# xinyiW915/ReLaX-VQA

Measured on AMD Instinct MI355X. Metric: clips/sec (32 sampled frames, 1080p) feature extraction, higher is better.
Workload: dtype f32 (fp32-grade split-operand arithmetic, fp32 accumulate: the whole ViT (GEMMs and attention), ResNet-50's stem, layer3 / layer4, and in layer1 / layer2 the 3x3 convolutions, every conv3 (back to back with its 3x3), the downsample convolutions and layer2's conv1 on fp32 operands as 2 fp16 planes x

## Files before the change

### relax-vqa_amd/csrc/gemm_h2.hip

```cpp
#include "relax_internal.h"
#include "host_logic.h"
#include "h2.h"
#include "gelu.h"

#ifndef H3_EP_FETCH_AHEAD
#define H3_EP_FETCH_AHEAD 0
#endif
#ifndef H2_STAMP
#define H2_STAMP(i_)
#define H2_STAMPS_BEFORE_LAUNCH(h_, p_, units_)
#define H2_STAMPS_AFTER_LAUNCH(h_, p_, units_, s_)
#endif
#ifndef H3_ABL_NO_A
#define H3_ABL_NO_A(taps_, perimg_, p_) false
#define H3_ABL_NO_OUT_H2(taps_, p_) false
#endif
#ifndef H3_KSTEP
#define H3_KSTEP(k_) (k_)
#endif

namespace relax {

typedef float h2k_f32x4 __attribute__((ext_vector_type(4)));
typedef float f32x4 __attribute__((ext_vector_type(4)));
// ... 168 lines not shown
    {
        const int per_group = p.group_m * p.tiles_n;
        const int g = tile / per_group;
        const int first = g * p.group_m;
        const int gsz = p.tiles_m - first < p.group_m ? p.tiles_m - first : p.group_m;
        const int w = tile - g * per_group;
        tm = first + w % gsz;
        tn = w / gsz;
    }
    const int m0 = tm * BM;
    const int n0 = tn * BN;
    H2_STAMP(0);

    const int64_t row_bytes = (int64_t)p.K * 4;
    __amdgpu_buffer_rsrc_t rsrc_a, rsrc_w;
    {
        const int64_t left = (int64_t)(p.M - m0) * row_bytes;
        rsrc_a = __builtin_amdgcn_make_buffer_rsrc(const_cast<char*>(p.a + (int64_t)m0 * row_bytes), 0,
                                                   (int)(left < kH2MaxRecords ? left : kH2MaxRecords), 0x00020000);
        rsrc_w = __builtin_amdgcn_make_buffer_rsrc(const_cast<char*>(p.w + (int64_t)n0 * row_bytes), 0, (int)(BN * row_bytes), 0x00020000);
    }
    unsigned voff_a, voff_w;
    {
        const int r = 32 * wave + (lane >> 1);
        voff_a = m0 + r < p.M ? (unsigned)(r * (int)row_bytes + (lane & 1) * 16) : kH2OutOfRange;
        voff_w = (unsigned)(r * (int)row_bytes + (lane & 1) * 16);
    }
    int d_kt = kt_begin;
#define H2_ISSUE_PIECE(st_, j_)                                                                                         \
    {                                                                                                                   \
        const int soff_ = d_kt * kH2ChunkBytes + ((j_) >> 1) * 32;                                                      \
        const int dst_ = (st_) * STAGE + ((j_) >> 1) * (STAGE / 2) + ((j_) & 1) * (BM * 32) + wave * 1024;               \
        if (((j_) & 1) == 0) { H2_DMA(rsrc_a, dst_, voff_a, soff_); }                                                    \
        else { H2_DMA(rsrc_w, dst_, voff_w, soff_); }                                                                    \
    }
#define H2_ISSUE(st_)                                                                                                   \
    {                                                                                                                   \
        _Pragma("unroll") for (int j = 0; j < PPW; ++j) H2_ISSUE_PIECE(st_, j);                                         \
        ++d_kt;                                                                                                         \
    }

    floatx4 acc[8][4];
#pragma unroll
    for (int i = 0; i < 8; ++i)
#pragma unroll
        for (int j = 0; j < 4; ++j)
#pragma unroll
            for (int r = 0; r < 4; ++r) acc[i][j][r] = 0.f;

    const int r16 = lane & 15, g16 = lane >> 4;
    const int a_hl = (g16 >> 1) * (STAGE / 2) + (wm * 128 + r16) * 32 + ((g16 & 1) << 4);
    const int b_hh = (BM + wn * 64 + r16) * 32 + ((g16 & 1) << 4);
    h2k_f16x8 xb[2][4][2], ya[2];
#define H2_READ_XB(set_, sp_)                                                                                           \
    _Pragma("unroll") for (int y = 0; y < 4; ++y) {                                                                     \
        xb[set_][y][0] = *reinterpret_cast<const h2k_f16x8*>((sp_) + b_hh + y * 16 * 32);                               \
        xb[set_][y][1] = *reinterpret_cast<const h2k_f16x8*>((sp_) + b_hh + y * 16 * 32 + STAGE / 2);                   \
    }
#define H2_READ_A(buf_, e_, sp_)                                                                                        \
    {                                                                                                                   \
        ya[buf_] = *reinterpret_cast<const h2k_f16x8*>((sp_) + a_hl + (e_) * 16 * 32);                                  \
        __builtin_amdgcn_sched_barrier(0);                        \
    }
#define H2_MFMAS(set_, buf_, e_)                                                                                        \
    {                                                                                                                   \
        _Pragma("unroll") for (int y = 0; y < 4; ++y)                                                                   \
            acc[e_][y] = __builtin_amdgcn_mfma_f32_16x16x32_f16(ya[buf_], xb[set_][y][1], acc[e_][y], 0, 0, 0);         \
        _Pragma("unroll") for (int y = 0; y < 4; ++y)                                                                   \
            acc[e_][y] = __builtin_amdgcn_mfma_f32_16x16x32_f16(ya[buf_], xb[set_][y][0], acc[e_][y], 0, 0, 0);         \
        __builtin_amdgcn_sched_barrier(0);        \
    }
#define H2_REGION(xs_, st_, has_next_, has_d_)                                                                          \
    {                                                                                                                   \
        const char* sn_ = smem + (((st_) + 1) % NSTG) * STAGE;                                                          \
        if (has_next_) {                                                                                                \
            if (has_d_) asm volatile("s_waitcnt vmcnt(%0) lgkmcnt(0)" ::"n"((NSTG - 2) * PPW) : "memory");              \
            else asm volatile("s_waitcnt vmcnt(0) lgkmcnt(0)" ::: "memory");                                            \
            __builtin_amdgcn_s_barrier();                                                                               \
            H2_READ_XB((xs_) ^ 1, sn_);                                                                                 \
            H2_READ_A(0, 0, sn_);                                                                                       \
        }                                                                                                               \
        H2_MFMAS(xs_, 1, 7);                                                                                            \
        if (has_next_) {                                                                                                \
            _Pragma("unroll") for (int e = 0; e < 7; ++e) {                                                             \
                H2_READ_A((e + 1) & 1, e + 1, sn_);                                                                     \
                if ((has_d_) && e < PPW) H2_ISSUE_PIECE(st_, e);                                                        \
                H2_MFMAS((xs_) ^ 1, e & 1, e);                                                                          \
            }                                                                                                           \
            if (has_d_) ++d_kt;                                                                                         \
        }                                                                                                               \
    }

    const int nk = kt_end - kt_begin;
    {
        const int pre = nk < NSTG ? nk : NSTG;
        for (int i = 0; i < pre; ++i) H2_ISSUE(i);
        if (pre >= 4) asm volatile("s_waitcnt vmcnt(%0)" ::"n"(3 * PPW) : "memory");
        else if (pre == 3) asm volatile("s_waitcnt vmcnt(%0)" ::"n"(2 * PPW) : "memory");
        else if (pre == 2) asm volatile("s_waitcnt vmcnt(%0)" ::"n"(PPW) : "memory");
        else asm volatile("s_waitcnt vmcnt(0)" ::: "memory");
    }
    __builtin_amdgcn_s_barrier();
    H2_READ_XB(0, smem);
    H2_READ_A(0, 0, smem);
    H2_STAMP(1);
#pragma unroll
    for (int e = 0; e < 7; ++e) {
        H2_READ_A((e + 1) & 1, e + 1, smem);
        H2_MFMAS(0, e & 1, e);
    }
    {
        constexpr int PERIOD = (NSTG % 2 == 0) ? NSTG : 2 * NSTG;
        int k = 0;
        for (; k + PERIOD + NSTG <= nk; k += PERIOD) {
#pragma unroll
            for (int i = 0; i < PERIOD; ++i) H2_REGION(i & 1, i % NSTG, true, true);
        }
        for (; k < nk; k += PERIOD) {
#pragma unroll
            for (int i = 0; i < PERIOD; ++i)
                if (k + i < nk) H2_REGION(i & 1, i % NSTG, k + i + 1 < nk, k + i + NSTG < nk);
        }
    }
#undef H2_REGION
#undef H2_MFMAS
#undef H2_READ_A
#undef H2_READ_XB
#undef H2_ISSUE
#undef H2_ISSUE_PIECE
    H2_STAMP(2);
    __syncthreads();

    float* stg = reinterpret_cast<float*>(smem);
    constexpr int LDC = BN + 4;
    constexpr int EP_ROWS = 64;
    constexpr int C8 = BN / 8;
    constexpr int NT = 512;
    static_assert(EP_ROWS * LDC * 4 <= NSTG * STAGE, "epilogue pass must fit the staging LDS");
    constexpr int EP_STEP = NT / C8;
    constexpr int EP_ITERS = EP_ROWS / EP_STEP;
    const bool planes = p.out_h2 != nullptr;
    const int lcA = planes ? (tid % C8) * 8 : (tid % C8) * 4;
    const int lcB = planes ? lcA + 4 : lcA + BN / 2;
    const int lr0 = tid / C8;
    const f32x4 zero4 = {0.f, 0.f, 0.f, 0.f};
    f32x4 bias_a = zero4, bias_b = zero4, cs_a = zero4, cs_b = zero4;
    if (slice < 0) {
        cs_a = *reinterpret_cast<const f32x4*>(p.colscale + n0 + lcA);
        cs_b = *reinterpret_cast<const f32x4*>(p.colscale + n0 + lcB);
        if (p.bias) {
            bias_a = *reinterpret_cast<const f32x4*>(p.bias + n0 + lcA);
            bias_b = *reinterpret_cast<const f32x4*>(p.bias + n0 + lcB);
        }
    }
    const bool interior = m0 + BM <= p.M;
#pragma unroll
    for (int pass = 0; pass < BM / EP_ROWS; ++pass) {
        if (pass > 0) __syncthreads();
        f32x4 ra[EP_ITERS], rb[EP_ITERS];
        float rs[EP_ITERS];
#pragma unroll
        for (int it = 0; it < EP_ITERS; ++it) {
            const int m = m0 + pass * EP_ROWS + it * EP_STEP + lr0;
            ra[it] = zero4;
            rb[it] = zero4;
            rs[it] = 1.f;
            if (slice < 0 && (interior || m < p.M)) {
                if (p.residual) {
                    const float* r = p.residual + (int64_t)m * p.N + n0;
                    ra[it] = *reinterpret_cast<const f32x4*>(r + lcA);
                    rb[it] = *reinterpret_cast<const f32x4*>(r + lcB);
                }
                if (p.rowscale) rs[it] = p.rowscale[m];
            }
        }
#pragma unroll
        for (int x = 0; x < 8; ++x) {
            const int rb0 = wm * 128 + x * 16;
            if (rb0 / EP_ROWS == pass) {
#pragma unroll
                for (int y = 0; y < 4; ++y)
#pragma unroll
                    for (int r = 0; r < 4; ++r) stg[(rb0 % EP_ROWS + 4 * g16 + r) * LDC + wn * 64 + y * 16 + r16] = acc[x][y][r];
            }
        }
        __syncthreads();
#pragma unroll
        for (int it = 0; it < EP_ITERS; ++it) {
            const int lr = it * EP_STEP + lr0;
            const int trow = pass * EP_ROWS + lr;
            const int m = m0 + trow;
            if (!interior && m >= p.M) continue;
            f32x4 va = *reinterpret_cast<const f32x4*>(stg + lr * LDC + lcA);
            f32x4 vb = *reinterpret_cast<const f32x4*>(stg + lr * LDC + lcB);
            if (slice >= 0) {
                float* o = p.partial + ((int64_t)split_tile * p.nsplit + slice) * (BM * BN) + (int64_t)trow * BN;
                *reinterpret_cast<f32x4*>(o + lcA) = va;
                *reinterpret_cast<f32x4*>(o + lcB) = vb;
                continue;
            }
            va = va * (cs_a * rs[it]) + bias_a;
            vb = vb * (cs_b * rs[it]) + bias_b;
            if (p.residual) {
                va += ra[it];
                vb += rb[it];
            }
            if (p.act == 1) {
                va = (f32x4){fmaxf(va.x, 0.f), fmaxf(va.y, 0.f), fmaxf(va.z, 0.f), fmaxf(va.w, 0.f)};
                vb = (f32x4){fmaxf(vb.x, 0.f), fmaxf(vb.y, 0.f), fmaxf(vb.z, 0.f), fmaxf(vb.w, 0.f)};
            } else if (p.act == 2) {
                va = gelu_erf4(va);
                vb = gelu_erf4(vb);
            }
            const int64_t o = (int64_t)m * p.N + n0;
            if (p.out) {
                *reinterpret_cast<f32x4*>(p.out + o + lcA) = va;
                *reinterpret_cast<f32x4*>(p.out + o + lcB) = vb;
            }
            if (p.out_h2) store_h2_x8(p.out_h2 + (int64_t)m * ((int64_t)p.N * 4), n0 + lcA, va, vb, p.out_scale);
        }
    }
    H2_STAMP(3);
#endif
}

constexpr int H3_OPSTAGE = H2_BM * 128;
static_assert(H2_BM == H2_BN, "gemm_h3: the operand rings share their stage size");
#ifndef H3_PLAIN_STAGES
#define H3_PLAIN_STAGES 3, 2, 0
#endif
#ifndef H3_CONV1_STAGES
#define H3_CONV1_STAGES 2, 2, 0
#endif
#ifndef H3_TAPS_STAGES
#define H3_TAPS_STAGES 2, 2, 0
#endif
struct H3Rings { int a, b, order; };
constexpr H3Rings h3_rings(bool taps, bool perimg) { return taps ? H3Rings{H3_TAPS_STAGES} : perimg ? H3Rings{H3_CONV1_STAGES} : H3Rings{H3_PLAIN_STAGES}; }
constexpr size_t h3_lds_bytes(bool taps, bool perimg) { return (size_t)(h3_rings(taps, perimg).a + h3_rings(taps, perimg).b) * H3_OPSTAGE; }
#ifndef H2_STAMP_LATCH
#define H2_STAMP_LATCH(v_)
#define H2_STAMP_PUT(i_, v_)
#endif

__device__ inline float dpp_row_max(float v) {
#define H3_DPP_MAX(CTRL_) v = fmaxf(v, __builtin_bit_cast(float, __builtin_amdgcn_update_dpp(0, __builtin_bit_cast(int, v), CTRL_, 0xf, 0xf, true)))
    H3_DPP_MAX(0xB1);
    H3_DPP_MAX(0x4E);
    H3_DPP_MAX(0x141);
    H3_DPP_MAX(0x140);
#undef H3_DPP_MAX
    return v;
}

#if __HIP_DEVICE_COMPILE__
template <bool FOUR, bool TAPS, bool PERIMG, int ASTG, int BSTG, int ORDER>
__device__ __forceinline__ void gemm_h3_body(const H2Params& p) {
    constexpr int BM = H2_BM, BN = H2_BN, OPSTG = H3_OPSTAGE, IMG = OPSTG / 2, B0 = ASTG * OPSTG;
    constexpr int LA = ASTG - 2, LB = BSTG - 2;
    static_assert(LA >= 0 && LB >= 0 && LA + LB <= 1 && (ORDER == 0 || ORDER == 1), "gemm_h3: 2 + 2, 3 + 2 or 2 + 3 stages");
    constexpr int WAITN = ORDER == 0 ? 4 : 2;
    extern __shared__ __attribute__((aligned(16))) char smem[];
    const int tid = threadIdx.x;
    const int lane = tid & 63;
    const int wave = __builtin_amdgcn_readfirstlane(tid >> 6);
    const int wm = wave >> 2, wn = wave & 3;

    int tile, kt_begin, kt_end, slice = -1, split_tile = 0;
    {
        const int nk_all = p.K >> 5;
        const int b = blockIdx.x;
        if (b < p.full_tiles) {
            tile = xcd_remap_h2(b, p.full_tiles);
            kt_begin = 0;
            kt_end = nk_all;
        } else {
            const int u = b - p.full_tiles;
            split_tile = u / p.nsplit;
            slice = u - split_tile * p.nsplit;
            tile = p.full_tiles + split_tile;
            kt_begin = (int)((int64_t)nk_all * slice / p.nsplit);
            kt_end = (int)((int64_t)nk_all * (slice + 1) / p.nsplit);
        }
    }
    int tm, tn;
    {
        const int per_group = p.group_m * p.tiles_n;
        const int g = tile / per_group;
        const int first = g * p.group_m;
        const int gsz = p.tiles_m - first < p.group_m ? p.tiles_m - first : p.group_m;
        const int w = tile - g * per_group;
        tm = first + w % gsz;
        tn = w / gsz;
    }
    const int m0 = tm * BM;
    const int n0 = tn * BN;
#ifdef H3_STAGGER
    if (PERIMG && !TAPS && blockIdx.x < 256 && (blockIdx.x & 3)) {
        const unsigned long long t0 = __builtin_amdgcn_s_memtime(), wait = (unsigned long long)(blockIdx.x & 3) * (H3_STAGGER);
        while (__builtin_amdgcn_s_memtime() - t0 < wait) __builtin_amdgcn_s_sleep(32);
    }
#endif
    H2_STAMP(0);

    const int64_t row_bytes = (int64_t)p.K * 4;
    const int64_t arow_bytes = p.pixels ? (int64_t)p.Cin * 4 : row_bytes;
    const int img0 = p.pixels ? m0 / (p.Ho * p.Wo) : 0;
    __amdgpu_buffer_rsrc_t rsrc_a, rsrc_w;
    {
        const int64_t base = p.pixels ? (int64_t)img0 * p.H * p.W * arow_bytes : (int64_t)m0 * arow_bytes;
        const int64_t total = p.pixels ? (int64_t)(p.M / (p.Ho * p.Wo)) * p.H * p.W * arow_bytes : (int64_t)p.M * arow_bytes;
        const int64_t left = total - base;
        rsrc_a = __builtin_amdgcn_make_buffer_rsrc(const_cast<char*>(p.a + base), 0, (int)(left < kH2MaxRecords ? left : kH2MaxRecords), 0x00020000);
        rsrc_w = __builtin_amdgcn_make_buffer_rsrc(const_cast<char*>(p.w + (int64_t)n0 * row_bytes), 0, (int)(BN * row_bytes), 0x00020000);
    }
    unsigned voff[4];
    [[maybe_unused]] unsigned a_taps[2] = {0u, 0u};
    const int ntaps = TAPS ? p.K / p.Cin : 1;
#pragma unroll
    for (int q = 0; q < 4; ++q) {
        const int trow = (wave + 8 * q) * 16 + (lane >> 2);
        const int unit = (lane & 3) ^ ((4 - ((trow >> 2) & 3)) & 3);
        const int off = (unit >> 1) * kH2ChunkBytes + (unit & 1) * 16;
        if (q >= 2) {
            voff[q] = (unsigned)((trow - BM) * (int)row_bytes + off);
        } else if (m0 + trow >= p.M || H3_ABL_NO_A(TAPS, PERIMG, p)) {
            voff[q] = kH2OutOfRange;
        } else if (p.pixels) {
            const int m = m0 + trow;
            const int img = m / (p.Ho * p.Wo);
            const int rem = m - img * (p.Ho * p.Wo);
            const int oy = rem / p.Wo;
            const int ox = rem - oy * p.Wo;
            const int iy = oy * p.stride - p.pad, ix = ox * p.stride - p.pad;
            if (TAPS) {
                for (int t = 0, dy = 0, dx = 0; t < ntaps; ++t) {
                    if ((unsigned)(iy + dy) < (unsigned)p.H && (unsigned)(ix + dx) < (unsigned)p.W) a_taps[q] |= 1u << t;
                    if (++dx == p.KW) { dx = 0; ++dy; }
                }
            }
            voff[q] = (unsigned)((((img - img0) * p.H + iy) * p.W + ix) * (int)arow_bytes + off);
        } else {
            voff[q] = (unsigned)(trow * (int)arow_bytes + off);
        }
    }
    int dA_kt = kt_begin;
    [[maybe_unused]] int dA_cc = 0, dA_tap = 0, dA_dy = 0, dA_dx = 0;
    [[maybe_unused]] const int cin_chunks = p.Cin >> 4;
    if (TAPS) {
        dA_cc = kt_begin / ntaps;
        dA_tap = kt_begin - dA_cc * ntaps;
        dA_dy = dA_tap / p.KW;
        dA_dx = dA_tap - dA_dy * p.KW;
    }
    [[maybe_unused]] int dW_kt_own = dA_kt, dW_cc_own = dA_cc, dW_tap_own = dA_tap;
    int &dW_kt = LA + LB > 0 ? dW_kt_own : dA_kt, &dW_cc = LA + LB > 0 ? dW_cc_own : dA_cc, &dW_tap = LA + LB > 0 ? dW_tap_own : dA_tap;
#define H3_ISSUE_A(st_, i_)                                                                                             \
    {                                                                                                                   \
        const int dst_ = (st_) * OPSTG + ((i_) >> 1) * IMG + (wave + 8 * ((i_) & 1)) * 1024;                             \
        if (TAPS) {                                                                                                     \
            const bool ok_ = (a_taps[(i_) & 1] >> dA_tap) & 1u;                                                         \
            const int tapoff_ = (dA_dy * p.W + dA_dx) * (int)arow_bytes + dA_cc * (2 * kH2ChunkBytes) + ((i_) >> 1) * 32; \
            H2_DMA(rsrc_a, dst_, ok_ ? voff[(i_) & 1] + (unsigned)tapoff_ : kH2OutOfRange, 0);                          \
        } else {                                                                                                        \
            H2_DMA(rsrc_a, dst_, voff[(i_) & 1], H3_KSTEP(dA_kt) * (2 * kH2ChunkBytes) + ((i_) >> 1) * 32);             \
        }                                                                                                               \
    }
#define H3_ISSUE_W(st_, i_)                                                                                             \
    {                                                                                                                   \
        const int dst_ = B0 + (st_) * OPSTG + ((i_) >> 1) * IMG + (wave + 8 * ((i_) & 1)) * 1024;                        \
        const int wk_ = TAPS ? (dW_tap * cin_chunks + 2 * dW_cc) * kH2ChunkBytes : H3_KSTEP(dW_kt) * (2 * kH2ChunkBytes); \
        H2_DMA(rsrc_w, dst_, voff[2 + ((i_) & 1)], wk_ + ((i_) >> 1) * 32);                                              \
    }
#define H3_ADVANCE_A()                                                                                                  \
    {                                                                                                                   \
        ++dA_kt;                                                                                                        \
        if (TAPS) {                                                                                                     \
            ++dA_tap;                                                                                                   \
            ++dA_dx;                                                                                                    \
            const bool wx_ = dA_dx == p.KW;                                                                             \
            dA_dx = wx_ ? 0 : dA_dx;                                                                                    \
            dA_dy += wx_ ? 1 : 0;                                                                                       \
            const bool wt_ = dA_tap == ntaps;                                                                           \
            dA_tap = wt_ ? 0 : dA_tap;                                                                                  \
            dA_dy = wt_ ? 0 : dA_dy;                                                                                    \
            dA_cc += wt_ ? 1 : 0;                                                                                       \
        }                                                                                                               \
    }
#define H3_ADVANCE_W()                                                                                                  \
    if (LA + LB > 0) {                                                                                                  \
        ++dW_kt;                                                                                                        \
        if (TAPS) {                                                                                                     \
            ++dW_tap;                                                                                                   \
            const bool wt_ = dW_tap == ntaps;                                                                           \
            dW_tap = wt_ ? 0 : dW_tap;                                                                                  \
            dW_cc += wt_ ? 1 : 0;                                                                                       \
        }                                                                                                               \
    }
#define H3_ISSUE_SLOT(sa_, sb_, s_, has_a_, has_b_)                                                                     \
    {                                                                                                                   \
        const bool grouped_ = LA + LB > 0 && ORDER == 0;                                                                \
        const bool second_ = grouped_ ? (s_) >= 4 : ((s_) & 3) >= 2;                \
        const bool is_a_ = LA + LB == 0 ? !second_ : second_ == (LA == 1);      \
        const int i_ = grouped_ ? (s_) & 3 : ((s_) >> 2) * 2 + ((s_) & 1);                                              \
        if (is_a_) {                                                                                                    \
            if (has_a_) H3_ISSUE_A(sa_, i_);                                                                            \
        } else {                                                                                                        \
            if (has_b_) H3_ISSUE_W(sb_, i_);                                                                            \
        }                                                                                                               \
    }
#define H3_ISSUE_STEP_A(step_)                                                                                          \
    {                                                                                                                   \
        _Pragma("unroll") for (int i = 0; i < 4; ++i) H3_ISSUE_A((step_) % ASTG, i);                                    \
        H3_ADVANCE_A();                                                                                                 \
    }
#define H3_ISSUE_STEP_W(step_)                                                                                          \
    {                                                                                                                   \
        _Pragma("unroll") for (int i = 0; i < 4; ++i) H3_ISSUE_W((step_) % BSTG, i);                                    \
        H3_ADVANCE_W();                                                                                                 \
    }

    floatx4 acc[8][4];
#pragma unroll
    for (int i = 0; i < 8; ++i)
#pragma unroll
        for (int j = 0; j < 4; ++j)
#pragma unroll
            for (int r = 0; r < 4; ++r) acc[i][j][r] = 0.f;

    const int r16 = lane & 15, g16 = lane >> 4;
    const int f16 = (4 - ((r16 >> 2) & 3)) & 3;
    const int a_h = (wm * 128 + r16) * 64 + ((g16 ^ f16) << 4);
    const int b_h = (wn * 64 + r16) * 64 + ((g16 ^ f16) << 4);
    h2k_f16x8 xb[2][4][2], ya[2][2];
#define H3_READ_XB(set_, sp_)                                                                                           \
    _Pragma("unroll") for (int y = 0; y < 4; ++y) {                                                                     \
        xb[set_][y][0] = *reinterpret_cast<const h2k_f16x8*>((sp_) + b_h + y * 16 * 64);                                \
        xb[set_][y][1] = *reinterpret_cast<const h2k_f16x8*>((sp_) + b_h + y * 16 * 64 + IMG);                          \
    }
#define H3_READ_A(buf_, e_, sp_)                                                                                        \
    {                                                                                                                   \
        ya[buf_][0] = *reinterpret_cast<const h2k_f16x8*>((sp_) + a_h + (e_) * 16 * 64);                                \
        ya[buf_][1] = *reinterpret_cast<const h2k_f16x8*>((sp_) + a_h + (e_) * 16 * 64 + IMG);                          \
        __builtin_amdgcn_sched_barrier(0);                      \
    }
#define H3_MFMAS(set_, buf_, e_)                                                                                        \
    {                                                                                                                   \
        if (FOUR) {                                                                                                     \
            _Pragma("unroll") for (int y = 0; y < 4; ++y)                                                               \
                acc[e_][y] = __builtin_amdgcn_mfma_f32_16x16x32_f16(ya[buf_][1], xb[set_][y][1], acc[e_][y], 0, 0, 0);  \
        }                                                                                                               \
        _Pragma("unroll") for (int y = 0; y < 4; ++y)                                                                   \
            acc[e_][y] = __builtin_amdgcn_mfma_f32_16x16x32_f16(ya[buf_][1], xb[set_][y][0], acc[e_][y], 0, 0, 0);      \
        _Pragma("unroll") for (int y = 0; y < 4; ++y)                                                                   \
            acc[e_][y] = __builtin_amdgcn_mfma_f32_16x16x32_f16(ya[buf_][0], xb[set_][y][1], acc[e_][y], 0, 0, 0);      \
        _Pragma("unroll") for (int y = 0; y < 4; ++y)                                                                   \
            acc[e_][y] = __builtin_amdgcn_mfma_f32_16x16x32_f16(ya[buf_][0], xb[set_][y][0], acc[e_][y], 0, 0, 0);      \
        __builtin_amdgcn_sched_barrier(0);        \
    }
#define H3_REGION(k6_, has_next_, has_e_, has_l_)                                                                       \
    {                                                                                                                   \
        const char* sa_ = smem + (((k6_) + 1) % ASTG) * OPSTG;                                                          \
        const char* sb_ = smem + B0 + (((k6_) + 1) % BSTG) * OPSTG;                                                     \
        const bool has_a_ = LA ? (has_l_) : (has_e_), has_b_ = LB ? (has_l_) : (has_e_);                                \
        if (has_next_) {                                                                                                \
            if (LA + LB > 0 && (has_e_)) asm volatile("s_waitcnt vmcnt(%0) lgkmcnt(0)" ::"n"(WAITN) : "memory");        \
            else asm volatile("s_waitcnt vmcnt(0) lgkmcnt(0)" ::: "memory");                                            \
            __builtin_amdgcn_s_barrier();                                                                               \
            H3_READ_XB(((k6_) + 1) & 1, sb_);                                                                           \
            H3_READ_A(0, 0, sa_);                                                                                       \
            H3_ISSUE_SLOT(((k6_) + 2 + LA) % ASTG, ((k6_) + 2 + LB) % BSTG, 0, has_a_, has_b_);                         \
        }                                                                                                               \
        H3_MFMAS((k6_) & 1, 1, 7);                                                                                      \
        if (has_next_) {                                                                                                \
            _Pragma("unroll") for (int e = 0; e < 7; ++e) {                                                             \
                H3_READ_A((e + 1) & 1, e + 1, sa_);                                                                     \
                H3_ISSUE_SLOT(((k6_) + 2 + LA) % ASTG, ((k6_) + 2 + LB) % BSTG, e + 1, has_a_, has_b_);                 \
                H3_MFMAS(((k6_) + 1) & 1, e & 1, e);                                                                    \
            }                                                                                                           \
            if (has_a_) H3_ADVANCE_A();                                                                                 \
            if (has_b_) H3_ADVANCE_W();                                                                                 \
        }                                                                                                               \
    }

    const int nk = kt_end - kt_begin;
    if (LA + LB == 0) {
#pragma unroll
        for (int j = 0; j < 8; ++j) H3_ISSUE_SLOT(0, 0, j, true, true);
        H3_ADVANCE_A();
        H3_ADVANCE_W();
        if (nk > 1) {
#pragma unroll
            for (int j = 0; j < 8; ++j) H3_ISSUE_SLOT(1, 1, j, true, true);
            H3_ADVANCE_A();
            H3_ADVANCE_W();
            asm volatile("s_waitcnt vmcnt(8)" ::: "memory");
        } else {
            asm volatile("s_waitcnt vmcnt(0)" ::: "memory");
        }
    } else {
        if (LA) {
            H3_ISSUE_STEP_W(0);
            H3_ISSUE_STEP_A(0);
        } else {
            H3_ISSUE_STEP_A(0);
            H3_ISSUE_STEP_W(0);
        }
        if (nk > 1) {
            if (LA) {
                H3_ISSUE_STEP_W(1);
                H3_ISSUE_STEP_A(1);
            } else {
                H3_ISSUE_STEP_A(1);
                H3_ISSUE_STEP_W(1);
            }
        }
        if (nk > 2) {
            if (LA) H3_ISSUE_STEP_A(2) else H3_ISSUE_STEP_W(2)
            asm volatile("s_waitcnt vmcnt(12)" ::: "memory");
        } else if (nk > 1) {
            asm volatile("s_waitcnt vmcnt(8)" ::: "memory");
        } else {
            asm volatile("s_waitcnt vmcnt(0)" ::: "memory");
        }
    }
    __builtin_amdgcn_s_barrier();
    H3_READ_XB(0, smem + B0);
    H3_READ_A(0, 0, smem);
    H2_STAMP_LATCH(stamp1);
#pragma unroll
    for (int e = 0; e < 7; ++e) {
        H3_READ_A((e + 1) & 1, e + 1, smem);
        H3_MFMAS(0, e & 1, e);
    }
    {
        constexpr int PERIOD = LA + LB > 0 ? 6 : 2;
        int k = 0;
        for (; k + PERIOD + 1 + LA + LB < nk; k += PERIOD) {
#pragma unroll
            for (int i = 0; i < PERIOD; ++i) H3_REGION(i, true, true, true);
        }
        for (; k < nk; k += PERIOD) {
#pragma unroll
            for (int i = 0; i < PERIOD; ++i)
                if (k + i < nk) H3_REGION(i, k + i + 1 < nk, k + i + 2 < nk, k + i + 3 < nk);
        }
    }
#undef H3_REGION
#undef H3_ISSUE_STEP_W
#undef H3_ISSUE_STEP_A
#undef H3_ISSUE_SLOT
#undef H3_ADVANCE_W
#undef H3_ADVANCE_A
#undef H3_ISSUE_W
#undef H3_ISSUE_A
#undef H3_MFMAS
#undef H3_READ_A
#undef H3_READ_XB
    H2_STAMP_PUT(1, stamp1);
    H2_STAMP(2);
    __syncthreads();
    H2_STAMP(7);

    float* stg = reinterpret_cast<float*>(smem);
    constexpr int LDC = BN + 4;
    constexpr int EP_ROWS = 64;
    constexpr int C8 = BN / 8;
    constexpr int NT = 512;
    static_assert(EP_ROWS * LDC * 4 <= 96 * 1024 && 96 * 1024 + 64 <= (ASTG + BSTG) * OPSTG, "epilogue pass must fit the staging LDS");
    constexpr int EP_STEP = NT / C8;
    constexpr int EP_ITERS = EP_ROWS / EP_STEP;
    const bool planes = p.out_h2 != nullptr || (PERIMG && p.residual_h2 != nullptr);
    const int lcA = planes ? (tid % C8) * 8 : (tid % C8) * 4;
    const int lcB = planes ? lcA + 4 : lcA + BN / 2;
    const int lr0 = tid / C8;
    const f32x4 zero4 = {0.f, 0.f, 0.f, 0.f};
    const f32x4 cs_a = *reinterpret_cast<const f32x4*>(p.colscale + n0 + lcA);
    const f32x4 cs_b = *reinterpret_cast<const f32x4*>(p.colscale + n0 + lcB);
    const __amdgpu_buffer_rsrc_t rs_bias = __builtin_amdgcn_make_buffer_rsrc(const_cast<float*>(p.bias), 0, p.bias ? p.N * 4 : 0, 0x00020000);
    const f32x4 bias_a = __builtin_bit_cast(f32x4, __builtin_amdgcn_raw_buffer_load_b128(rs_bias, (n0 + lcA) * 4, 0, 0));
    const f32x4 bias_b = __builtin_bit_cast(f32x4, __builtin_amdgcn_raw_buffer_load_b128(rs_bias, (n0 + lcB) * 4, 0, 0));
    const bool interior = m0 + BM <= p.M;
    unsigned* simg = reinterpret_cast<unsigned*>(smem + 96 * 1024);
    const int rpi = p.rows_per_img;
    const int img_first = rpi > 0 ? m0 / rpi : 0;
    const int row_first = m0 - img_first * rpi;
    const float rpi_inv = rpi > 0 ? 1.f / (float)rpi : 0.f;
    auto img_of_row = [&](int trow) -> int {
        const int x = row_first + trow;
        int q = (int)((float)x * rpi_inv);
        q -= (q * rpi > x) ? 1 : 0;
        q += ((q + 1) * rpi <= x) ? 1 : 0;
        return img_first + q;
    };
    const bool lds_amax = PERIMG && p.amax_out && slice < 0 && p.rows_per_img >= 18;
    if (lds_amax && tid < 16) simg[tid] = 0u;
    const int64_t tile_ofs = ((int64_t)m0 * p.N + n0) * 4;
    const unsigned row_pitch = (unsigned)p.N * 4u;
    const unsigned ofs_f = (unsigned)lr0 * row_pitch + (unsigned)lcA * 4u;
    const unsigned ofs_p = (unsigned)lr0 * row_pitch + (unsigned)h2_offset(lcA);
    const unsigned ofs_fb = (unsigned)(lcB - lcA) * 4u;
    const bool res_planes = PERIMG && p.residual_h2 != nullptr;
    const char* res_ptr = res_planes ? p.residual_h2 : reinterpret_cast<const char*>(p.residual);
    const int64_t res_left = (int64_t)p.M * p.N * 4 - tile_ofs;
    const __amdgpu_buffer_rsrc_t rs_res = __builtin_amdgcn_make_buffer_rsrc(
        const_cast<char*>(res_ptr) + (res_ptr ? tile_ofs : 0), 0, (res_ptr && slice < 0) ? (int)(res_left < kH2MaxRecords ? res_left : kH2MaxRecords) : 0, 0x00020000);
    const unsigned ofs_r = res_planes ? ofs_p : ofs_f, ofs_rb = res_planes ? 32u : ofs_fb;
    char* tile_out = reinterpret_cast<char*>(p.out) + tile_ofs;
    char* tile_out_h2 = p.out_h2 + tile_ofs;
    f32x4 ra[EP_ITERS], rb[EP_ITERS];
    float rs[EP_ITERS], os[EP_ITERS], rri[EP_ITERS];
    int im[EP_ITERS];
#define H3_EP_FETCH(P_, IT_)                                                                                                     \
    {                                                                                                                            \
        const int trow_ = (P_) * EP_ROWS + (IT_) * EP_STEP + lr0;                                                                \
        const int m_ = m0 + trow_;                                                                                               \
        const unsigned row_ofs_ = (unsigned)(((P_) * EP_ROWS + (IT_) * EP_STEP) * row_pitch);                                    \
        ra[IT_] = __builtin_bit_cast(f32x4, __builtin_amdgcn_raw_buffer_load_b128(rs_res, row_ofs_ + ofs_r, 0, 0));              \
        rb[IT_] = __builtin_bit_cast(f32x4, __builtin_amdgcn_raw_buffer_load_b128(rs_res, row_ofs_ + ofs_r + ofs_rb, 0, 0));     \
        rs[IT_] = 1.f;                                                                                                           \
        os[IT_] = p.out_scale;                                                                                                   \
        rri[IT_] = 1.f;                                                                                                          \
        im[IT_] = 0;                                                                                                             \
        if (slice < 0 && (interior || m_ < p.M)) {                                                                               \
            if (p.rowscale) rs[IT_] = p.rowscale[m_];                                                                            \
            if (PERIMG && rpi > 0) {                                                      \
                im[IT_] = img_of_row(trow_);                                                                                     \
                if (p.img_in_inv) rs[IT_] = p.img_in_inv[im[IT_]];                                                               \
                if (p.img_out_scale) os[IT_] = p.img_out_scale[im[IT_]];                                                         \
            }                                                                                                                    \
            if (res_planes) rri[IT_] = p.img_res_inv[im[IT_]];  \
        }                                                                                                                        \
    }
    constexpr bool EP_AHEAD = PERIMG && H3_EP_FETCH_AHEAD;
    if constexpr (EP_AHEAD) {
#pragma unroll
        for (int it = 0; it < EP_ITERS; ++it) H3_EP_FETCH(0, it);
    }
#pragma unroll
    for (int pass = 0; pass < BM / EP_ROWS; ++pass) {
        if (pass > 0) __syncthreads();
        if constexpr (!EP_AHEAD) {
#pragma unroll
            for (int it = 0; it < EP_ITERS; ++it) H3_EP_FETCH(pass, it);
        }
        if (pass == 0) H2_STAMP(4);
#pragma unroll
        for (int x = 0; x < 8; ++x) {
            const int rb0 = wm * 128 + x * 16;
            if (rb0 / EP_ROWS == pass) {
#pragma unroll
                for (int y = 0; y < 4; ++y)
#pragma unroll
                    for (int r = 0; r < 4; ++r) stg[(rb0 % EP_ROWS + 4 * g16 + r) * LDC + wn * 64 + y * 16 + r16] = acc[x][y][r];
            }
        }
        __syncthreads();
        if (pass == 0) H2_STAMP(5);
        if constexpr (!EP_AHEAD) {
#pragma unroll
            for (int it = 0; it < EP_ITERS; ++it) {
                asm volatile("" : "+v"(ra[it]), "+v"(rb[it]), "+v"(rs[it]));
                if constexpr (PERIMG) asm volatile("" : "+v"(os[it]), "+v"(rri[it]));
            }
        }
#pragma unroll
        for (int it = 0; it < EP_ITERS; ++it) {
            const int lr = it * EP_STEP + lr0;
            const int trow = pass * EP_ROWS + lr;
            const int m = m0 + trow;
            f32x4 xa = ra[it], xb = rb[it];
            const float rs_it = rs[it], os_it = os[it];
            const int im_it = im[it];
            if (res_planes) {
                const h2_u32x4 hi = __builtin_bit_cast(h2_u32x4, xa), lo = __builtin_bit_cast(h2_u32x4, xb);
                const float ri = rri[it];
#define H2_LO16(u_) ((float)__builtin_bit_cast(_Float16, (unsigned short)((u_) & 0xffffu)))
#define H2_HI16(u_) ((float)__builtin_bit_cast(_Float16, (unsigned short)((u_) >> 16)))
                xa = (f32x4){H2_LO16(hi.x) + H2_LO16(lo.x), H2_HI16(hi.x) + H2_HI16(lo.x), H2_LO16(hi.y) + H2_LO16(lo.y),
                             H2_HI16(hi.y) + H2_HI16(lo.y)} * ri;
                xb = (f32x4){H2_LO16(hi.z) + H2_LO16(lo.z), H2_HI16(hi.z) + H2_HI16(lo.z), H2_LO16(hi.w) + H2_LO16(lo.w),
                             H2_HI16(hi.w) + H2_HI16(lo.w)} * ri;
#undef H2_LO16
#undef H2_HI16
            }
            if constexpr (EP_AHEAD) {
                if (pass + 1 < BM / EP_ROWS) H3_EP_FETCH(pass + 1, it);
            }
            if (!interior && m >= p.M) continue;
            f32x4 va = *reinterpret_cast<const f32x4*>(stg + lr * LDC + lcA);
            f32x4 vb = *reinterpret_cast<const f32x4*>(stg + lr * LDC + lcB);
            if (slice >= 0) {
                float* o = p.partial + ((int64_t)split_tile * p.nsplit + slice) * (BM * BN) + (int64_t)trow * BN;
                *reinterpret_cast<f32x4*>(o + lcA) = va;
                *reinterpret_cast<f32x4*>(o + lcB) = vb;
                continue;
            }
            va = va * (cs_a * rs_it) + bias_a;
            vb = vb * (cs_b * rs_it) + bias_b;
            if (res_ptr) {
                va += xa;
                vb += xb;
            }
            if (p.act == 1) {
                va = (f32x4){fmaxf(va.x, 0.f), fmaxf(va.y, 0.f), fmaxf(va.z, 0.f), fmaxf(va.w, 0.f)};
                vb = (f32x4){fmaxf(vb.x, 0.f), fmaxf(vb.y, 0.f), fmaxf(vb.z, 0.f), fmaxf(vb.w, 0.f)};
            } else if (p.act == 2) {
                va = gelu_erf4(va);
                vb = gelu_erf4(vb);
            }
            const unsigned row_ofs = (unsigned)((pass * EP_ROWS + it * EP_STEP) * row_pitch);
            if (p.out && (!PERIMG || m < p.out_rows)) {
                char* o = tile_out + (size_t)(unsigned)(row_ofs + ofs_f);
                *reinterpret_cast<f32x4*>(o) = va;
                *reinterpret_cast<f32x4*>(o + ofs_fb) = vb;
            }
            if (PERIMG && p.gap) {
                *reinterpret_cast<f32x4*>(stg + lr * LDC + lcA) = va;
                *reinterpret_cast<f32x4*>(stg + lr * LDC + lcB) = vb;
            }
            if (p.out_h2 && !H3_ABL_NO_OUT_H2(TAPS, p)) {
                h2_u32x4 hi, lo;
                split2_x8(va * os_it, vb * os_it, hi, lo);
                char* o = tile_out_h2 + (size_t)(unsigned)(row_ofs + ofs_p);
                *reinterpret_cast<h2_u32x4*>(o) = hi;
                *reinterpret_cast<h2_u32x4*>(o + 32) = lo;
            }
            if (PERIMG && p.amax_out) {
                float mx = fmaxf(fmaxf(fmaxf(va.x, va.y), fmaxf(va.z, va.w)), fmaxf(fmaxf(vb.x, vb.y), fmaxf(vb.z, vb.w)));
                mx = dpp_row_max(mx);
                if ((tid & 15) == 0) {
                    if (lds_amax) atomicMax(simg + (im_it - img_first), __float_as_uint(mx));
                    else atomicMax(p.amax_out + im_it, __float_as_uint(mx));
                }
            }
        }
        if (pass == 0) H2_STAMP(6);
        if (PERIMG && p.gap && slice < 0) {
            __syncthreads();
            for (int e = tid; e < (EP_ROWS / 4) * BN; e += NT) {
                const int g = e / BN, col = e - g * BN;
                const int mg = m0 + pass * EP_ROWS + g * 4;
                if (mg < p.gap_rows) {
                    float t = 0.f;
#pragma unroll
                    for (int r = 0; r < 4; ++r) t += stg[(g * 4 + r) * LDC + col];
                    p.gap[(int64_t)(mg >> 2) * p.N + n0 + col] = t;
                }
            }
        }
    }
#undef H3_EP_FETCH
    if (lds_amax) {
        __syncthreads();
        if (tid < 16 && simg[tid] != 0u) atomicMax(p.amax_out + img_first + tid, simg[tid]);
    }
    H2_STAMP(3);
}
#endif

template <bool FOUR, bool TAPS = false, bool PERIMG = false>
__global__ __launch_bounds__(512, 2) void gemm_h3(const H2Params p) {
#if __HIP_DEVICE_COMPILE__
    constexpr H3Rings R = h3_rings(TAPS, PERIMG);
    gemm_h3_body<FOUR, TAPS, PERIMG, R.a, R.b, R.order>(p);
#endif
}

__global__ __launch_bounds__(256) void splitk_finish_h2(const H2Params p) {
    constexpr int BM = H2_BM, BN = H2_BN;
    const int split_tile = blockIdx.y;
    const int tile = p.full_tiles + split_tile;
    int tm, tn;
    {
        const int per_group = p.group_m * p.tiles_n;
        const int g = tile / per_group;
        const int first = g * p.group_m;
        const int gsz = p.tiles_m - first < p.group_m ? p.tiles_m - first : p.group_m;
        const int w = tile - g * per_group;
        tm = first + w % gsz;
        tn = w / gsz;
    }
    const int m0 = tm * BM;
    const int n0 = tn * BN;
    const int e8 = blockIdx.x * 256 + threadIdx.x;
    const int lr = e8 / (BN / 8), lc = (e8 % (BN / 8)) * 8;
    const int m = m0 + lr;
    __shared__ unsigned s_mx[8];
    const int img_b0 = p.rows_per_img > 0 ? (m0 + blockIdx.x * 8) / p.rows_per_img : 0;
    if (threadIdx.x < 8) s_mx[threadIdx.x] = 0u;
    __syncthreads();
    if (m < p.M) {
    const float* pt = p.partial + (int64_t)split_tile * p.nsplit * (BM * BN) + lr * BN + lc;
    f32x4 va = *reinterpret_cast<const f32x4*>(pt), vb = *reinterpret_cast<const f32x4*>(pt + 4);
    for (int k = 1; k < p.nsplit; ++k) {
        va += *reinterpret_cast<const f32x4*>(pt + (int64_t)k * (BM * BN));
        vb += *reinterpret_cast<const f32x4*>(pt + (int64_t)k * (BM * BN) + 4);
    }
    const int64_t o = (int64_t)m * p.N + n0 + lc;
    float rs = p.rowscale ? p.rowscale[m] : 1.f, os = p.out_scale;
    const int img = p.rows_per_img > 0 ? m / p.rows_per_img : 0;
    if (p.rows_per_img > 0) {
        if (p.img_in_inv) rs = p.img_in_inv[img];
        if (p.img_out_scale) os = p.img_out_scale[img];
    }
    va = va * (*reinterpret_cast<const f32x4*>(p.colscale + n0 + lc) * rs);
    vb = vb * (*reinterpret_cast<const f32x4*>(p.colscale + n0 + lc + 4) * rs);
    if (p.bias) {
        va += *reinterpret_cast<const f32x4*>(p.bias + n0 + lc);
        vb += *reinterpret_cast<const f32x4*>(p.bias + n0 + lc + 4);
    }
    if (p.residual) {
        va += *reinterpret_cast<const f32x4*>(p.residual + o);
        vb += *reinterpret_cast<const f32x4*>(p.residual + o + 4);
    }
    if (p.act == 1) {
        va = (f32x4){fmaxf(va.x, 0.f), fmaxf(va.y, 0.f), fmaxf(va.z, 0.f), fmaxf(va.w, 0.f)};
        vb = (f32x4){fmaxf(vb.x, 0.f), fmaxf(vb.y, 0.f), fmaxf(vb.z, 0.f), fmaxf(vb.w, 0.f)};
    } else if (p.act == 2) {
        va = gelu_erf4(va);
        vb = gelu_erf4(vb);
    }
    if (p.out && m < p.out_rows) {
        *reinterpret_cast<f32x4*>(p.out + o) = va;
        *reinterpret_cast<f32x4*>(p.out + o + 4) = vb;
    }
    if (p.out_h2) store_h2_x8(p.out_h2 + (int64_t)m * ((int64_t)p.N * 4), n0 + lc, va, vb, os);
    if (p.amax_out) {
        float mx = fmaxf(fmaxf(fmaxf(va.x, va.y), fmaxf(va.z, va.w)), fmaxf(fmaxf(vb.x, vb.y), fmaxf(vb.z, vb.w)));
#pragma unroll
        for (int o = 16; o >= 1; o >>= 1) mx = fmaxf(mx, __shfl_xor(mx, o));
        if ((threadIdx.x & 31) == 0) atomicMax(&s_mx[(img - img_b0) & 7], __float_as_uint(mx));
    }
    }
    if (p.amax_out) {
        __syncthreads();
        if (threadIdx.x < 8 && s_mx[threadIdx.x] != 0u) atomicMax(p.amax_out + img_b0 + threadIdx.x, s_mx[threadIdx.x]);
    }
}

template <int FORM>
static int launch_h2_variant(relax_handle* h, H2Params& p, hipStream_t s) {
    constexpr int BM = H2_BM, BN = H2_BN;
    constexpr bool BK32 = FORM >= 2;
    const bool can_split = h->gemm.split_k && !p.no_split && !p.gap && !p.residual_h2;
    RELAX_TRY(plan_tiles(h, p, BM, BN, 256, BK32 ? p.K / 32 : p.K / 16, BK32 ? 4 : 8, can_split));
    constexpr size_t lds = BK32 ? h3_lds_bytes(FORM == 4, FORM >= 4) : (size_t)(FORM == 1 ? 4 : 3) * H2_STAGE;
    auto kernel = [] {
        if constexpr (FORM == 0) return &gemm_h2<3>;
        else if constexpr (FORM == 1) return &gemm_h2<4>;
        else if constexpr (FORM == 2) return &gemm_h3<false>;
        else if constexpr (FORM == 3) return &gemm_h3<true>;
        else if constexpr (FORM == 4) return &gemm_h3<false, true, true>;
        else return &gemm_h3<false, false, true>;
    }();
    static std::atomic<bool> lds_allowed[kMaxDevices];
    RELAX_TRY(allow_dynamic_lds(h, {reinterpret_cast<const void*>(kernel)}, lds, lds_allowed));
    const int units = p.full_tiles + (p.ntiles - p.full_tiles) * p.nsplit;
    H2_STAMPS_BEFORE_LAUNCH(h, p, units);
    hipLaunchKernelGGL(kernel, dim3(units), dim3(512), lds, s, p);
    H2_STAMPS_AFTER_LAUNCH(h, p, units, s);
    if (p.nsplit > 1)
        hipLaunchKernelGGL(splitk_finish_h2, dim3(BM * BN / 8 / 256, p.ntiles - p.full_tiles), dim3(256), 0, s, p);
    RELAX_HIP_CHECK(h, hipGetLastError());
    return RELAX_OK;
}

int launch_gemm_h2(relax_handle* h, const GemmDescH2& d, hipStream_t s) {
    H2Params p{};
    p.a = static_cast<const char*>(d.a);
    p.w = static_cast<const char*>(d.w);
    p.colscale = d.colscale; p.rowscale = d.rowscale;
    p.bias = d.bias; p.residual = d.residual; p.out = d.out; p.out_h2 = static_cast<char*>(d.out_h2); p.out_scale = d.out_scale;
    p.M = d.M; p.N = d.N; p.K = d.K; p.act = d.act; p.no_split = d.no_split;
    const bool conv = d.pixels != 0;
    const bool taps = conv && d.KH * d.KW > 1;
    if (conv) {
        p.pixels = 1; p.H = d.H; p.W = d.W; p.Cin = d.Cin; p.Ho = d.Ho; p.Wo = d.Wo; p.KW = d.KW; p.stride = d.stride; p.pad = d.pad;
        RELAX_REQUIRE(h, d.Nimg > 0 && d.M == d.Nimg * d.Ho * d.Wo && d.K == d.KH * d.KW * d.Cin && d.Cin % 32 == 0 && d.KH * d.KW <= 32 &&
                             (taps || d.pad == 0) && d.stride >= 1 && (int64_t)d.H * d.W * d.Cin * 4 * 4 < kH2MaxRecords,
                      "f16x2 conv: bad geometry (Cin=%d must be a multiple of 32, at most 32 taps, M = Nimg*Ho*Wo, K = KH*KW*Cin)", d.Cin);
    }
    p.rows_per_img = d.rows_per_img; p.img_in_inv = d.img_in_inv; p.img_out_scale = d.img_out_scale; p.amax_out = d.amax_out;
    p.residual_h2 = static_cast<const char*>(d.residual_h2); p.img_res_inv = d.img_res_inv; p.gap = d.gap_groups;
    p.out_rows = d.out_rows > 0 && d.out_rows < d.M ? d.out_rows : d.M;
    p.gap_rows = d.gap_rows > 0 && d.gap_rows < d.M ? d.gap_rows : d.M;
    RELAX_REQUIRE(h, !(d.residual && d.residual_h2) && (!d.residual_h2 || (d.img_res_inv && d.rows_per_img > 0)), "f16x2 gemm: bad residual");
    RELAX_REQUIRE(h, !d.gap_groups || (d.rows_per_img > 0 && d.rows_per_img % 4 == 0), "f16x2 conv: the fused spatial mean needs Ho*Wo %% 4 == 0");
    RELAX_REQUIRE(h, d.rows_per_img > 0 || (!d.img_in_inv && !d.img_out_scale && !d.amax_out), "f16x2 gemm: per-image tables need rows_per_img");
    RELAX_REQUIRE(h, conv || (d.rows_per_img == 0 && !d.residual_h2 && !d.gap_groups && d.out_rows == 0),
                  "f16x2 gemm: per-image scales, plane residuals, fused means and out_rows belong to the convolution form");
    RELAX_REQUIRE(h, p.M > 0 && p.N > 0 && p.K > 0, "f16x2 gemm: empty problem M=%d N=%d K=%d", p.M, p.N, p.K);
    RELAX_REQUIRE(h, p.K % 16 == 0 && p.N % 256 == 0, "f16x2 gemm: K=%d must be a multiple of 16 and N=%d of 256", p.K, p.N);
    RELAX_REQUIRE(h, (int64_t)p.K * 4 * 256 < kH2MaxRecords, "f16x2 gemm: K=%d too large", p.K);
    RELAX_REQUIRE(h, d.a && d.w && d.colscale && (d.out || d.out_h2 || d.gap_groups), "f16x2 gemm: missing operand / no output requested");
    RELAX_REQUIRE(h, !d.amax_out || d.act == 1, "f16x2 gemm: amax_out needs act == 1 (ReLU): the bit-ordered maximum is valid for non-negative outputs only");
    RELAX_REQUIRE(h, !d.out_h2 || d.img_out_scale || (d.out_scale > 0.f && d.out_scale < 3.0e38f), "f16x2 gemm: the plane output needs its scale");
    auto aligned16 = [](const void* q) { return (reinterpret_cast<uintptr_t>(q) & 15) == 0; };
    RELAX_REQUIRE(h, aligned16(d.a) && aligned16(d.w) && aligned16(d.colscale) && aligned16(d.bias) && aligned16(d.residual) && aligned16(d.out) &&
                         aligned16(d.out_h2),
                  "f16x2 gemm: every operand pointer must be 16-byte aligned");
    const double flops = 2.0 * p.M * (double)p.N * (double)p.K;
    const double bytes = 4.0 * ((conv ? (double)d.Nimg * d.H * d.W * d.Cin : (double)p.M * p.K) + (double)p.N * p.K) +
                         (double)p.M * p.N * ((d.out ? 4.0 : 0.0) + (d.out_h2 ? 4.0 : 0.0) + (d.residual ? 4.0 : 0.0));
    int span;
    RELAX_TRY(prof_begin(h, s, conv ? 5 : 6, flops, &span, bytes));
    int rc;
    if (conv) {
        RELAX_REQUIRE(h, p.K % 32 == 0, "f16x2 conv: K=%d must be a multiple of 32", p.K);
        rc = taps ? launch_h2_variant<4>(h, p, s) : launch_h2_variant<5>(h, p, s);
    } else if (h->gemm.h2_form == 0 || p.K % 32 != 0) rc = h->gemm.h2_stages == 4 ? launch_h2_variant<1>(h, p, s) : launch_h2_variant<0>(h, p, s);
    else if (h->gemm.h2_form == 2 || p.K < 256) rc = launch_h2_variant<3>(h, p, s);
    else rc = launch_h2_variant<2>(h, p, s);
    if (rc != RELAX_OK) { prof_abort(h, span); return rc; }
    RELAX_TRY(prof_end(h, s, span));
    return RELAX_OK;
}

}
```

Baseline: 119.0.

## Restructure conv epilogue: per-thread 4-row groups, LDS per-image tables, register-fused mean

In the convolution form of the epilogue, each thread now owns four consecutive rows, which are the aligned 4-row groups of the fused spatial mean. The mean is summed in registers and written as vector stores, replacing the LDS staging pass and its extra barrier. The per-image input, output and residual scale tables are prefetched at kernel start into LDS slots and read there, instead of gathered per row from global memory. The per-image amax is reduced per thread run and via DPP across the wavefront before fewer atomics. This changes the row-to-thread mapping and so the store coalescing pattern, uses more LDS, and adds an alignment requirement on the gap pointer.

```diff
diff --git a/relax-vqa_amd/csrc/gemm_h2.hip b/relax-vqa_amd/csrc/gemm_h2.hip
--- a/relax-vqa_amd/csrc/gemm_h2.hip
+++ b/relax-vqa_amd/csrc/gemm_h2.hip
@@ -494,6 +494,25 @@
     }
 #endif
     H2_STAMP(0);
+    const int rpi = p.rows_per_img;
+    const int img_first = rpi > 0 ? m0 / rpi : 0;
+    const int row_first = m0 - img_first * rpi;
+    const float rpi_inv = rpi > 0 ? 1.f / (float)rpi : 0.f;
+    const bool in_tab = PERIMG && rpi > 0 && p.img_in_inv != nullptr;
+    bool out_tab = false, res_tab = false;
+    float l_in = 0.f, l_out = 0.f, l_res = 0.f;
+    if constexpr (PERIMG) {
+        const int n_img = rpi > 0 ? (p.M - 1) / rpi + 1 : 1;
+        const int timg = img_first + (tid & (BM - 1)) < n_img ? img_first + (tid & (BM - 1)) : n_img - 1;
+        out_tab = rpi > 0 && p.img_out_scale != nullptr;
+        res_tab = p.residual_h2 != nullptr && p.img_res_inv != nullptr;
+        const __amdgpu_buffer_rsrc_t rs_tin = __builtin_amdgcn_make_buffer_rsrc(const_cast<float*>(p.img_in_inv), 0, in_tab ? n_img * 4 : 0, 0x00020000);
+        const __amdgpu_buffer_rsrc_t rs_tout = __builtin_amdgcn_make_buffer_rsrc(const_cast<float*>(p.img_out_scale), 0, out_tab ? n_img * 4 : 0, 0x00020000);
+        const __amdgpu_buffer_rsrc_t rs_tres = __builtin_amdgcn_make_buffer_rsrc(const_cast<float*>(p.img_res_inv), 0, res_tab ? n_img * 4 : 0, 0x00020000);
+        l_in = __builtin_bit_cast(float, __builtin_amdgcn_raw_buffer_load_b32(rs_tin, timg * 4, 0, 0));
+        l_out = __builtin_bit_cast(float, __builtin_amdgcn_raw_buffer_load_b32(rs_tout, timg * 4, 0, 0));
+        l_res = __builtin_bit_cast(float, __builtin_amdgcn_raw_buffer_load_b32(rs_tres, timg * 4, 0, 0));
+    }
 
     const int64_t row_bytes = (int64_t)p.K * 4;
     const int64_t arow_bytes = p.pixels ? (int64_t)p.Cin * 4 : row_bytes;
@@ -759,13 +778,17 @@
     constexpr int EP_ROWS = 64;
     constexpr int C8 = BN / 8;
     constexpr int NT = 512;
-    static_assert(EP_ROWS * LDC * 4 <= 96 * 1024 && 96 * 1024 + 64 <= (ASTG + BSTG) * OPSTG, "epilogue pass must fit the staging LDS");
+    constexpr int EP_SLOTS = BM;
+    static_assert(EP_ROWS * LDC * 4 <= 96 * 1024 && 96 * 1024 + 4 * EP_SLOTS * 4 <= (ASTG + BSTG) * OPSTG, "epilogue pass must fit the staging LDS");
     constexpr int EP_STEP = NT / C8;
     constexpr int EP_ITERS = EP_ROWS / EP_STEP;
     const bool planes = p.out_h2 != nullptr || (PERIMG && p.residual_h2 != nullptr);
     const int lcA = planes ? (tid % C8) * 8 : (tid % C8) * 4;
     const int lcB = planes ? lcA + 4 : lcA + BN / 2;
     const int lr0 = tid / C8;
+    constexpr int EP_RSTEP = PERIMG ? 1 : EP_STEP;
+    static_assert(!PERIMG || EP_ITERS == 4, "convolution form: a thread owns the aligned 4-row groups of the fused mean");
+    const int lrb = PERIMG ? EP_ITERS * lr0 : lr0;
     const f32x4 zero4 = {0.f, 0.f, 0.f, 0.f};
     const f32x4 cs_a = *reinterpret_cast<const f32x4*>(p.colscale + n0 + lcA);
     const f32x4 cs_b = *reinterpret_cast<const f32x4*>(p.colscale + n0 + lcB);
@@ -774,23 +797,29 @@
     const f32x4 bias_b = __builtin_bit_cast(f32x4, __builtin_amdgcn_raw_buffer_load_b128(rs_bias, (n0 + lcB) * 4, 0, 0));
     const bool interior = m0 + BM <= p.M;
     unsigned* simg = reinterpret_cast<unsigned*>(smem + 96 * 1024);
-    const int rpi = p.rows_per_img;
-    const int img_first = rpi > 0 ? m0 / rpi : 0;
-    const int row_first = m0 - img_first * rpi;
-    const float rpi_inv = rpi > 0 ? 1.f / (float)rpi : 0.f;
-    auto img_of_row = [&](int trow) -> int {
+    float* s_in = reinterpret_cast<float*>(simg + EP_SLOTS);
+    float* s_out = s_in + EP_SLOTS;
+    float* s_res = s_out + EP_SLOTS;
+    auto slot_of_row = [&](int trow) -> int {
+        if (rpi <= 0) return 0;
         const int x = row_first + trow;
         int q = (int)((float)x * rpi_inv);
         q -= (q * rpi > x) ? 1 : 0;
         q += ((q + 1) * rpi <= x) ? 1 : 0;
-        return img_first + q;
+        return q;
     };
-    const bool lds_amax = PERIMG && p.amax_out && slice < 0 && p.rows_per_img >= 18;
-    if (lds_amax && tid < 16) simg[tid] = 0u;
+    const bool tile_amax = PERIMG && p.amax_out && slice < 0;
+    float run_mx = 0.f;
+    int run_slot = PERIMG ? slot_of_row(lrb) : 0;
+    auto post_max = [&](int s, float v) {
+        v = dpp_row_max(v);
+        v = fmaxf(v, __builtin_bit_cast(float, __builtin_amdgcn_update_dpp(0, __builtin_bit_cast(int, v), 0x142, 0xa, 0xf, false)));
+        if ((tid & 31) == 31 && v != 0.f) atomicMax(simg + s, __float_as_uint(v));
+    };
     const int64_t tile_ofs = ((int64_t)m0 * p.N + n0) * 4;
     const unsigned row_pitch = (unsigned)p.N * 4u;
-    const unsigned ofs_f = (unsigned)lr0 * row_pitch + (unsigned)lcA * 4u;
-    const unsigned ofs_p = (unsigned)lr0 * row_pitch + (unsigned)h2_offset(lcA);
+    const unsigned ofs_f = (unsigned)lrb * row_pitch + (unsigned)lcA * 4u;
+    const unsigned ofs_p = (unsigned)lrb * row_pitch + (unsigned)h2_offset(lcA);
     const unsigned ofs_fb = (unsigned)(lcB - lcA) * 4u;
     const bool res_planes = PERIMG && p.residual_h2 != nullptr;
     const char* res_ptr = res_planes ? p.residual_h2 : reinterpret_cast<const char*>(p.residual);
@@ -801,27 +830,19 @@
     char* tile_out = reinterpret_cast<char*>(p.out) + tile_ofs;
     char* tile_out_h2 = p.out_h2 + tile_ofs;
     f32x4 ra[EP_ITERS], rb[EP_ITERS];
-    float rs[EP_ITERS], os[EP_ITERS], rri[EP_ITERS];
-    int im[EP_ITERS];
+    float rs[EP_ITERS], os[EP_ITERS];
 #define H3_EP_FETCH(P_, IT_)                                                                                                     \
     {                                                                                                                            \
-        const int trow_ = (P_) * EP_ROWS + (IT_) * EP_STEP + lr0;                                                                \
+        const int trow_ = (P_) * EP_ROWS + (IT_) * EP_RSTEP + lrb;                                                               \
         const int m_ = m0 + trow_;                                                                                               \
-        const unsigned row_ofs_ = (unsigned)(((P_) * EP_ROWS + (IT_) * EP_STEP) * row_pitch);                                    \
+        const unsigned row_ofs_ = (unsigned)(((P_) * EP_ROWS + (IT_) * EP_RSTEP) * row_pitch);                                   \
+                                                                \
         ra[IT_] = __builtin_bit_cast(f32x4, __builtin_amdgcn_raw_buffer_load_b128(rs_res, row_ofs_ + ofs_r, 0, 0));              \
         rb[IT_] = __builtin_bit_cast(f32x4, __builtin_amdgcn_raw_buffer_load_b128(rs_res, row_ofs_ + ofs_r + ofs_rb, 0, 0));     \
         rs[IT_] = 1.f;                                                                                                           \
         os[IT_] = p.out_scale;                                                                                                   \
-        rri[IT_] = 1.f;                                                                                                          \
-        im[IT_] = 0;                                                                                                             \
         if (slice < 0 && (interior || m_ < p.M)) {                                                                               \
             if (p.rowscale) rs[IT_] = p.rowscale[m_];                                                                            \
-            if (PERIMG && rpi > 0) {                                                      \
-                im[IT_] = img_of_row(trow_);                                                                                     \
-                if (p.img_in_inv) rs[IT_] = p.img_in_inv[im[IT_]];                                                               \
-                if (p.img_out_scale) os[IT_] = p.img_out_scale[im[IT_]];                                                         \
-            }                                                                                                                    \
-            if (res_planes) rri[IT_] = p.img_res_inv[im[IT_]];  \
         }                                                                                                                        \
     }
     constexpr bool EP_AHEAD = PERIMG && H3_EP_FETCH_AHEAD;
@@ -847,26 +868,36 @@
                     for (int r = 0; r < 4; ++r) stg[(rb0 % EP_ROWS + 4 * g16 + r) * LDC + wn * 64 + y * 16 + r16] = acc[x][y][r];
             }
         }
+        if constexpr (PERIMG) {
+            if (pass == 0 && tid < EP_SLOTS) {
+                simg[tid] = 0u;
+                s_in[tid] = in_tab ? l_in : 1.f;
+                s_out[tid] = out_tab ? l_out : p.out_scale;
+                s_res[tid] = res_tab ? l_res : 1.f;
+            }
+        }
         __syncthreads();
         if (pass == 0) H2_STAMP(5);
         if constexpr (!EP_AHEAD) {
 #pragma unroll
             for (int it = 0; it < EP_ITERS; ++it) {
                 asm volatile("" : "+v"(ra[it]), "+v"(rb[it]), "+v"(rs[it]));
-                if constexpr (PERIMG) asm volatile("" : "+v"(os[it]), "+v"(rri[it]));
-            }
-        }
+            }
+        }
+        int slot = PERIMG ? slot_of_row(pass * EP_ROWS + lrb) : 0;
+        f32x4 ga = zero4, gb = zero4;
 #pragma unroll
         for (int it = 0; it < EP_ITERS; ++it) {
-            const int lr = it * EP_STEP + lr0;
+            const int lr = it * EP_RSTEP + lrb;
             const int trow = pass * EP_ROWS + lr;
             const int m = m0 + trow;
+            if (PERIMG && rpi > 0 && it > 0) slot += ((slot + 1) * rpi <= row_first + trow) ? 1 : 0;
             f32x4 xa = ra[it], xb = rb[it];
-            const float rs_it = rs[it], os_it = os[it];
-            const int im_it = im[it];
+            const float rs_it = in_tab ? s_in[slot] : rs[it];
+            const float os_it = PERIMG ? s_out[slot] : os[it];
             if (res_planes) {
                 const h2_u32x4 hi = __builtin_bit_cast(h2_u32x4, xa), lo = __builtin_bit_cast(h2_u32x4, xb);
-                const float ri = rri[it];
+                const float ri = s_res[slot];
 #define H2_LO16(u_) ((float)__builtin_bit_cast(_Float16, (unsigned short)((u_) & 0xffffu)))
 #define H2_HI16(u_) ((float)__builtin_bit_cast(_Float16, (unsigned short)((u_) >> 16)))
                 xa = (f32x4){H2_LO16(hi.x) + H2_LO16(lo.x), H2_HI16(hi.x) + H2_HI16(lo.x), H2_LO16(hi.y) + H2_LO16(lo.y),
@@ -901,15 +932,15 @@
                 va = gelu_erf4(va);
                 vb = gelu_erf4(vb);
             }
-            const unsigned row_ofs = (unsigned)((pass * EP_ROWS + it * EP_STEP) * row_pitch);
+            const unsigned row_ofs = (unsigned)((pass * EP_ROWS + it * EP_RSTEP) * row_pitch);
             if (p.out && (!PERIMG || m < p.out_rows)) {
                 char* o = tile_out + (size_t)(unsigned)(row_ofs + ofs_f);
                 *reinterpret_cast<f32x4*>(o) = va;
                 *reinterpret_cast<f32x4*>(o + ofs_fb) = vb;
             }
             if (PERIMG && p.gap) {
-                *reinterpret_cast<f32x4*>(stg + lr * LDC + lcA) = va;
-                *reinterpret_cast<f32x4*>(stg + lr * LDC + lcB) = vb;
+                ga += va;
+                gb += vb;
             }
             if (p.out_h2 && !H3_ABL_NO_OUT_H2(TAPS, p)) {
                 h2_u32x4 hi, lo;
@@ -918,34 +949,31 @@
                 *reinterpret_cast<h2_u32x4*>(o) = hi;
                 *reinterpret_cast<h2_u32x4*>(o + 32) = lo;
             }
-            if (PERIMG && p.amax_out) {
-                float mx = fmaxf(fmaxf(fmaxf(va.x, va.y), fmaxf(va.z, va.w)), fmaxf(fmaxf(vb.x, vb.y), fmaxf(vb.z, vb.w)));
-                mx = dpp_row_max(mx);
-                if ((tid & 15) == 0) {
-                    if (lds_amax) atomicMax(simg + (im_it - img_first), __float_as_uint(mx));
-                    else atomicMax(p.amax_out + im_it, __float_as_uint(mx));
+            if (tile_amax) {
+                const float mx = fmaxf(fmaxf(fmaxf(va.x, va.y), fmaxf(va.z, va.w)), fmaxf(fmaxf(vb.x, vb.y), fmaxf(vb.z, vb.w)));
+                if (slot != run_slot) {
+                    post_max(run_slot, run_mx);
+                    run_slot = slot;
+                    run_mx = 0.f;
                 }
+                run_mx = fmaxf(run_mx, mx);
             }
         }
         if (pass == 0) H2_STAMP(6);
         if (PERIMG && p.gap && slice < 0) {
-            __syncthreads();
-            for (int e = tid; e < (EP_ROWS / 4) * BN; e += NT) {
-                const int g = e / BN, col = e - g * BN;
-                const int mg = m0 + pass * EP_ROWS + g * 4;
-                if (mg < p.gap_rows) {
-                    float t = 0.f;
-#pragma unroll
-                    for (int r = 0; r < 4; ++r) t += stg[(g * 4 + r) * LDC + col];
-                    p.gap[(int64_t)(mg >> 2) * p.N + n0 + col] = t;
-                }
+            const int mg = m0 + pass * EP_ROWS + lrb;
+            if (mg < p.gap_rows) {
+                float* g = p.gap + (int64_t)(mg >> 2) * p.N + n0;
+                *reinterpret_cast<f32x4*>(g + lcA) = ga;
+                *reinterpret_cast<f32x4*>(g + lcB) = gb;
             }
         }
     }
 #undef H3_EP_FETCH
-    if (lds_amax) {
+    if (tile_amax) {
+        post_max(run_slot, run_mx);
         __syncthreads();
-        if (tid < 16 && simg[tid] != 0u) atomicMax(p.amax_out + img_first + tid, simg[tid]);
+        if (tid < EP_SLOTS && simg[tid] != 0u) atomicMax(p.amax_out + img_first + tid, simg[tid]);
     }
     H2_STAMP(3);
 }
@@ -1090,7 +1118,7 @@
     RELAX_REQUIRE(h, !d.out_h2 || d.img_out_scale || (d.out_scale > 0.f && d.out_scale < 3.0e38f), "f16x2 gemm: the plane output needs its scale");
     auto aligned16 = [](const void* q) { return (reinterpret_cast<uintptr_t>(q) & 15) == 0; };
     RELAX_REQUIRE(h, aligned16(d.a) && aligned16(d.w) && aligned16(d.colscale) && aligned16(d.bias) && aligned16(d.residual) && aligned16(d.out) &&
-                         aligned16(d.out_h2),
+                         aligned16(d.out_h2) && aligned16(d.gap_groups),
                   "f16x2 gemm: every operand pointer must be 16-byte aligned");
     const double flops = 2.0 * p.M * (double)p.N * (double)p.K;
     const double bytes = 4.0 * ((conv ? (double)d.Nimg * d.H * d.W * d.Cin : (double)p.M * p.K) + (double)p.N * p.K) +
```

Result: no change. 119.2, median of 3 (+0.2%).
